# crisbodnar/text-to-image

Hardware: AMD Instinct MI355X
Metric: images/sec (G+D step) at 64x64 batch=64 (higher is better)
Workload: dtype f32; 1 GPU; wgancls 64x64 batch=64/GPU fp32, synthetic images + random 1024-d text embeddings, D step (+kt) then G step, Adam(b1=0,b2=0.9); global_batch=64, parallelism=dp1, launch=hipGraph replay (1 graph/iteration)

## Files before the change

text-to-image_amd/csrc/t2i_bgemm.hip:

```cpp
#include <hip/hip_runtime.h>
#include <stdint.h>

#include <type_traits>

#include "t2i_internal.h"

namespace t2i {

typedef float f32x16 __attribute__((ext_vector_type(16)));
typedef unsigned int u32x4 __attribute__((ext_vector_type(4)));

namespace {
constexpr int BK = 32;
constexpr int KSTRIDE = BK + 4;
constexpr unsigned OOB = 0xFFFFFFF0u;

template <int LAY, int WM, int WN, int NW = 4>
struct BSmem {
  static constexpr bool A_KIN = LAY != 2, B_KIN = LAY == 1;
  static constexpr int BM = 32 * (NW / 2) * WM, BN = 64 * WN;
  static constexpr int A_ELEMS = A_KIN ? BM * KSTRIDE : BK * BM;
  static constexpr int B_ELEMS = B_KIN ? BN * KSTRIDE : BK * BN;
  static constexpr int BYTES = 2 * (A_ELEMS + B_ELEMS) * 4;
};
// ... 702 lines not shown
          const float y1 = apply_act((z[r][1] + z[r][2]) + bs_, q.act, q.alpha);
          const size_t oh = (size_t)q.sr * (2 * ty + r) + ph, ow0 = (size_t)q.sr * (2 * tx) + pw;
          float* o = q.out + (((size_t)b * q.OH + oh) * q.OW + ow0) * p.N + n;
          o[0] = y0;
          o[(size_t)q.sr * p.N] = y1;
        }
      }
    }
#pragma unroll
    for (int i = 0; i < 9; ++i)
#pragma unroll
      for (int e = 0; e < 16; ++e) acc[i][e] = 0.f;
  }
}

hipError_t bgemm9_launch(int lay, const Bgemm9Params& q, hipStream_t stream) {
  if (lay != 0 && lay != 1) return hipErrorInvalidValue;
  const int bytes = lay == 0 ? BSmem<0, 1, 1, 4>::BYTES : BSmem<1, 1, 1, 4>::BYTES;
  const int per_xcd = (q.g.items + 7) / 8;
  int nslot = per_xcd < 32 * 2 ? per_xcd : 32 * 2;
  if (nslot < 1) nslot = 1;
  if (lay == 0) hipLaunchKernelGGL((bgemm9_kernel<0, false>), dim3(nslot * 8), dim3(256), bytes, stream, q);
  else if (q.dy) {
    constexpr int wbytes = BSmem<1, 1, 1, 4>::BYTES + W9_PARK_BYTES;
    static bool attr_done = false;
    if (!attr_done) {
      hipError_t e = hipFuncSetAttribute(reinterpret_cast<const void*>(bgemm9_kernel<1, true>), hipFuncAttributeMaxDynamicSharedMemorySize, wbytes);
      if (e != hipSuccess) return e;
      attr_done = true;
    }
// ... 39 lines not shown
```

text-to-image_amd/csrc/t2i_capi.hip:

```cpp
#include <hip/hip_runtime.h>
#include <atomic>
#include <initializer_list>
#include <stdarg.h>
#include <stdio.h>
#include <stdlib.h>
#include <string.h>

#include "t2i_internal.h"

namespace t2i {

static thread_local char g_err[512] = "";

void set_error(const char* fmt, ...) {
  va_list ap;
  va_start(ap, fmt);
  vsnprintf(g_err, sizeof(g_err), fmt, ap);
  va_end(ap);
}

size_t col_reduce_ws(int64_t rows, int C);
hipError_t col_reduce_launch(const void*, const void*, const float*, int64_t, int, float*, float*, int, void*, hipStream_t, bool in_bf16 = false);
hipError_t bn_stats_launch(const void*, int64_t, int, float*, float*, const float*, const float*, float, float, float*, float*, float*,
                           float*, float*, float*, void*, hipStream_t, bool x_bf16 = false);
// ... 160 lines not shown
    v.debug_plan = env_int("T2I_DEBUG_PLAN", 0);
    v.group_n = env_int("T2I_GROUP_N", 8);
    v.bf16_dma = env_int("T2I_BF16_DMA", 1);
    v.hft_boost = env_int("T2I_HFT_BOOST", 130);
    v.hft_ovh = env_int("T2I_HFT_OVH", 80);
    v.bgemm = env_int("T2I_BGEMM", 1);
    v.bgemm_tile = env_int("T2I_BGEMM_TILE", 0);
    v.bgemm_big_items = env_int("T2I_BGEMM_BIG_ITEMS", 2048);
    v.dma_ovh = env_int("T2I_DMA_OVH", 120);
    v.dma_split_us = env_int("T2I_DMA_SPLIT_US", 29);
    v.tile8_eff = env_int("T2I_TILE8_EFF", 0);
    v.colred_wgs = env_int("T2I_COLRED_WGS", 768);
    v.wino_fuse = env_int("T2I_WINO_FUSE", 1);
    v.wino_fuse_items = env_int("T2I_WINO_FUSE_ITEMS", 512);
    v.wino_fuse_xf = env_int("T2I_WINO_FUSE_XF", 1);
    v.bn_fuse = env_int("T2I_BN_FUSE", 1);
    v.colred_cap = env_int("T2I_COLRED_CAP", 192);
    v.bf16_waves = env_int("T2I_BF16_WAVES", 8);
    v.bf16_pair_tiles = env_int("T2I_BF16_PAIR_TILES", 0);
    v.pair_reduce = env_int("T2I_PAIR_REDUCE", 1);
    v.h_stats = env_int("T2I_H_STATS", 0);
    v.pair_cus = env_int("T2I_PAIR_CUS", 128);
    v.pair_max_px = env_int("T2I_PAIR_MAX_PX", 49152);
    v.pair = env_int("T2I_PAIR", 1);
    v.vec_epi = env_int("T2I_VEC_EPI", 1);
    v.batch_lin = env_int("T2I_BATCH_LIN", 1);
    v.no_ut = env_int("T2I_NO_UT", 0);
    v.no_thin = env_int("T2I_NO_THIN", 0);
    v.winograd = env_int("T2I_WINOGRAD", 1);
    v.winograd_minc = env_int("T2I_WINOGRAD_MINC", 128);
// ... 1604 lines not shown
long long t2i_stat(const char* key) {
  if (key && !strcmp(key, "pair_fused")) return g_stat_pair_fused.load();
  return -1;
}

int t2i_tuning_set(const char* key, double value) {
  if (!key) { set_error("t2i_tuning_set: null key"); return T2I_ERR_INVALID; }
  Tuning& t = tuning_mut();
  struct { const char* name; int* field; } ints[] = {
      {"force_tile", &t.force_tile}, {"force_splitk", &t.force_splitk}, {"debug_plan", &t.debug_plan}, {"group_n", &t.group_n},
      {"no_ut", &t.no_ut}, {"no_thin", &t.no_thin}, {"winograd", &t.winograd}, {"winograd_minc", &t.winograd_minc},
      {"winograd_maxhw", &t.winograd_maxhw}, {"winograd_k4s2", &t.winograd_k4s2}, {"winograd_k4s2_minc", &t.winograd_k4s2_minc},
      {"winograd_k4s2_bwd_minc", &t.winograd_k4s2_bwd_minc}, {"winograd_k4s2_bwdf", &t.winograd_k4s2_bwdf}, {"winograd_k4s2_minwork", &t.winograd_k4s2_minwork}, {"winograd_k4s2_minitems", &t.winograd_k4s2_minitems},
      {"adam_blocks", &t.adam_blocks}, {"max_chain", &t.max_chain}, {"bf16_operands", &t.bf16_operands},
      {"cache_refresh", &t.cache_refresh}, {"thin_parts", &t.thin_parts}, {"batch_lin", &t.batch_lin}, {"bgemm", &t.bgemm}, {"winograd_minwork", &t.winograd_minwork}, {"bf16_dma", &t.bf16_dma}, {"hft_boost", &t.hft_boost}, {"hft_ovh", &t.hft_ovh},
      {"bgemm_tile", &t.bgemm_tile}, {"bgemm_big_items", &t.bgemm_big_items}, {"vec_epi", &t.vec_epi}, {"pair", &t.pair}, {"pair_cus", &t.pair_cus}, {"h_stats", &t.h_stats}, {"pair_reduce", &t.pair_reduce}, {"bf16_waves", &t.bf16_waves}, {"bf16_pair_tiles", &t.bf16_pair_tiles}, {"colred_wgs", &t.colred_wgs}, {"colred_cap", &t.colred_cap}, {"bn_fuse", &t.bn_fuse}, {"wino_fuse", &t.wino_fuse}, {"wino_fuse_items", &t.wino_fuse_items}, {"wino_fuse_xf", &t.wino_fuse_xf}, {"tile8_eff", &t.tile8_eff}, {"dma_ovh", &t.dma_ovh}, {"dma_split_us", &t.dma_split_us}, {"pair_max_px", &t.pair_max_px}};
  for (auto& e : ints)
    if (!strcmp(key, e.name)) { *e.field = (int)value; return T2I_OK; }
  if (!strcmp(key, "split_cost")) { t.split_cost = value; return T2I_OK; }
  set_error("t2i_tuning_set: unknown key '%s'", key);
  return T2I_ERR_INVALID;
}

int t2i_kt_sgd(float* kt, const float* wdist_sums, float scale, float lr, t2i_stream_t stream) {
  if (!kt || !wdist_sums) { set_error("t2i_kt_sgd: bad argument"); return T2I_ERR_INVALID; }
  return check(kt_sgd_launch(kt, wdist_sums, scale, lr, (hipStream_t)stream), "t2i_kt_sgd");
}

int t2i_zero_ranges(float* base, const int64_t* ranges, int32_t n, t2i_stream_t stream) {
  if (!base || !ranges || n <= 0) { set_error("t2i_zero_ranges: bad argument"); return T2I_ERR_INVALID; }
  return check(zero_ranges_launch(base, reinterpret_cast<const long long*>(ranges), n, (hipStream_t)stream), "t2i_zero_ranges");
// ... 383 lines not shown
```

text-to-image_amd/csrc/t2i_internal.h:

```cpp
#ifndef T2I_INTERNAL_H
#define T2I_INTERNAL_H

#include <hip/hip_runtime.h>
#include <stddef.h>
#include <stdint.h>

#include "../../include/t2i_hip.h"

namespace t2i {

enum { MODE_FWD = 0, MODE_BWD_DATA = 1, MODE_BWD_FILTER = 2 };

struct FastDiv {
  uint32_t mul, shr, add;
  __host__ void set(uint32_t d) {
    if (d == 1) { mul = 0; shr = 0; add = 0xFFFFFFFFu; return; }
    add = 0;
    uint32_t l = 0;
    while ((1u << l) < d) ++l;
    uint64_t pw = 1ull << (31 + l);
    mul = (uint32_t)((pw + d - 1) / d);
    shr = l - 1;
  }
  __host__ __device__ __forceinline__ int div(int n) const {
// ... 124 lines not shown
  uint32_t a_bytes, b_bytes;
};
hipError_t bgemm_launch(int lay, int wm, int wn, const BgemmParams& p, hipStream_t stream);
struct Bgemm9Params {
  BgemmParams g;
  const float* bias;
  float* out;
  int32_t OH, OW, Th, Tw;
  int32_t sr;
  int32_t act;
  float alpha;
  const float* dy;
  int32_t dHo, dWo;
};
hipError_t bgemm9_launch(int lay, const Bgemm9Params& q, hipStream_t stream);

struct Tuning {
  int force_tile, force_splitk, debug_plan, group_n, no_ut, no_thin;
  int winograd, winograd_minc, winograd_maxhw, winograd_k4s2, winograd_k4s2_minc, winograd_k4s2_bwd_minc, winograd_k4s2_bwdf;
  int adam_blocks, max_chain, bf16_operands, cache_refresh, thin_parts, batch_lin, bgemm, winograd_minwork, bf16_dma, hft_boost, hft_ovh, bgemm_tile, bgemm_big_items, vec_epi, pair, pair_cus, pair_max_px, dma_ovh, dma_split_us, tile8_eff, colred_wgs, colred_cap, h_stats, pair_reduce, bf16_waves, bf16_pair_tiles, bn_fuse, wino_fuse, wino_fuse_items, wino_fuse_xf, winograd_k4s2_minwork, winograd_k4s2_minitems;
  double split_cost;
};
const Tuning& tuning();

}
#endif
```

text-to-image_amd/csrc/t2i_winograd.hip:

```cpp
#include <hip/hip_runtime.h>
#include <stdint.h>
#include <stdio.h>
#include <string.h>
#include <stdlib.h>

#include <mutex>
#include <vector>

#include "t2i_internal.h"

namespace t2i {

struct FilterEntry {
  const float* w; int kind, Cin, Cout; float* U; size_t bytes; unsigned long long cap; hipStream_t stream; bool valid;
  hipStream_t cap_fill = nullptr;
};
static std::mutex g_fc_mu;
static std::vector<FilterEntry> g_fc;
static int g_fc_on = 0;
static char* g_fc_buf = nullptr;
static size_t g_fc_cap = 0, g_fc_used = 0;

int filter_cache_attach(void* buf, size_t bytes) {
  std::lock_guard<std::mutex> lk(g_fc_mu);
// ... 100 lines not shown
#pragma unroll
    for (int r = 0; r < 4; ++r) {
      const float u0 = s[r][0], u1 = 0.5f * (s[r][0] + s[r][1] + s[r][2]), u2 = 0.5f * (s[r][0] - s[r][1] + s[r][2]), u3 = s[r][2];
      U[((size_t)(r * 4 + 0) * K + k) * N + n] = u0;
      U[((size_t)(r * 4 + 1) * K + k) * N + n] = u1;
      U[((size_t)(r * 4 + 2) * K + k) * N + n] = u2;
      U[((size_t)(r * 4 + 3) * K + k) * N + n] = u3;
    }
  }
}

__global__ __launch_bounds__(256) void wino_filter_kernel(const float* __restrict__ w, int Cin, int Cout, float* __restrict__ U) {
  wino_filter_body(w, Cin, Cout, U, blockIdx.x, gridDim.x);
}

__device__ __forceinline__ int wino_slot(int r, int c, int flip) {
  const int rr = (flip && (r == 0 || r == 3)) ? 3 - r : r, cc = (flip && (c == 0 || c == 3)) ? 3 - c : c;
  return rr * 4 + cc;
}

__global__ __launch_bounds__(256) void wino_input_kernel(const float* __restrict__ x, int H, int W, int C, int Th, int Tw,
                                                         size_t T, float* __restrict__ V, int flip, size_t plane_T) {
  const int C4 = C >> 2;
  const size_t total = T * C4;
  for (size_t i = (size_t)blockIdx.x * blockDim.x + threadIdx.x; i < total; i += (size_t)gridDim.x * blockDim.x) {
    const int c4 = (int)(i % C4);
    const size_t t = i / C4;
    const int tx = (int)(t % Tw);
    const int ty = (int)((t / Tw) % Th);
    const size_t b = t / ((size_t)Tw * Th);
    float4 d[4][4];
// ... 16 lines not shown
      tt[2][c] = f4sub(d[2][c], d[1][c]);
      tt[3][c] = f4sub(d[1][c], d[3][c]);
    }
    float4* o = reinterpret_cast<float4*>(V) + t * C4 + c4;
    const size_t plane = plane_T * C4;
#pragma unroll
    for (int r = 0; r < 4; ++r) {
      wst(&o[(size_t)wino_slot(r, 0, flip) * plane], f4sub(tt[r][0], tt[r][2]));
      wst(&o[(size_t)wino_slot(r, 1, flip) * plane], f4add(tt[r][1], tt[r][2]));
      wst(&o[(size_t)wino_slot(r, 2, flip) * plane], f4sub(tt[r][2], tt[r][1]));
      wst(&o[(size_t)wino_slot(r, 3, flip) * plane], f4sub(tt[r][1], tt[r][3]));
    }
  }
}

__global__ __launch_bounds__(256) void wino_output_kernel(const float* __restrict__ Mx, const float* __restrict__ bias, int H,
                                                          int W, int N, int Th, int Tw, size_t T, int act, float alpha,
                                                          float* __restrict__ y, int flip) {
  const int N4 = N >> 2;
  const size_t total = T * N4;
  const size_t plane = T * N4;
  for (size_t i = (size_t)blockIdx.x * blockDim.x + threadIdx.x; i < total; i += (size_t)gridDim.x * blockDim.x) {
    const int n4 = (int)(i % N4);
    const size_t t = i / N4;
    const int tx = (int)(t % Tw);
    const int ty = (int)((t / Tw) % Th);
    const size_t b = t / ((size_t)Tw * Th);
    const float4* m = reinterpret_cast<const float4*>(Mx) + t * N4 + n4;
    float4 z[2][4];
#pragma unroll
    for (int c = 0; c < 4; ++c) {
      const float4 m0 = m[(size_t)wino_slot(0, c, flip) * plane], m1 = m[(size_t)wino_slot(1, c, flip) * plane],
                   m2 = m[(size_t)wino_slot(2, c, flip) * plane], m3 = m[(size_t)wino_slot(3, c, flip) * plane];
      z[0][c] = f4add(f4add(m0, m1), m2);
      z[1][c] = f4sub(f4sub(m1, m2), m3);
    }
    const float4 bs = bias ? reinterpret_cast<const float4*>(bias)[n4] : make_float4(0.f, 0.f, 0.f, 0.f);
#pragma unroll
    for (int r = 0; r < 2; ++r) {
      float4 y0 = f4add(f4add(f4add(z[r][0], z[r][1]), z[r][2]), bs);
      float4 y1 = f4add(f4sub(f4sub(z[r][1], z[r][2]), z[r][3]), bs);
      y0.x = apply_act(y0.x, act, alpha); y0.y = apply_act(y0.y, act, alpha); y0.z = apply_act(y0.z, act, alpha); y0.w = apply_act(y0.w, act, alpha);
      y1.x = apply_act(y1.x, act, alpha); y1.y = apply_act(y1.y, act, alpha); y1.z = apply_act(y1.z, act, alpha); y1.w = apply_act(y1.w, act, alpha);
      float4* o = reinterpret_cast<float4*>(y + ((b * H + 2 * ty + r) * W + 2 * tx) * N) + n4;
      o[0] = y0;
      o[N4] = y1;
// ... 10 lines not shown
  const int cmin = d.Cin < d.Cout ? d.Cin : d.Cout;
  const int maxhw = tuning().winograd_maxhw;
  if (cmin < wino_min_channels() || (int64_t)d.H * d.W > maxhw) return false;
  const int64_t T = (int64_t)d.B * (d.H / 2) * (d.W / 2);
  return T * d.Cin * d.Cout >= (int64_t)tuning().winograd_minwork;
}

bool winograd_filter_eligible(const t2i_conv_desc& d) {
  return winograd_eligible(d, false) && (int64_t)d.Cin * d.Cout >= 65536;
}

static void wino_dims(const t2i_conv_desc& d, bool bwd, size_t* T, int* K, int* N) {
  *T = (size_t)d.B * (d.H / 2) * (d.W / 2);
  *K = bwd ? d.Cout : d.Cin;
  *N = bwd ? d.Cin : d.Cout;
}

size_t winograd_ws(const t2i_conv_desc& d, bool bwd) {
  size_t T; int K, N;
  wino_dims(d, bwd, &T, &K, &N);
  return al256((size_t)16 * K * N * 4) + al256(16 * T * K * 4) + al256(16 * T * N * 4);
}

int winograd_conv(const t2i_conv_desc& d, bool bwd, const float* in, const float* w, const float* bias, float* out, int act,
                  float alpha, void* ws, size_t ws_bytes, hipStream_t stream, float* Vkeep) {
  size_t T; int K, N;
  wino_dims(d, bwd, &T, &K, &N);
  if (!ws || ws_bytes < winograd_ws(d, bwd) || (reinterpret_cast<uintptr_t>(ws) & 15)) {
    set_error("winograd conv: workspace %zu B < %zu B required (or misaligned)", ws_bytes, winograd_ws(d, bwd));
    return T2I_ERR_WORKSPACE;
  }
  char* base = reinterpret_cast<char*>(ws);
  float* U = reinterpret_cast<float*>(base);
  float* V = Vkeep ? Vkeep : reinterpret_cast<float*>(base + al256((size_t)16 * K * N * 4));
  float* Mx = reinterpret_cast<float*>(base + al256((size_t)16 * K * N * 4) + al256(16 * T * K * 4));
  const int Th = d.H / 2, Tw = d.W / 2;
  bool fill = true;
  if (float* Uc = filter_cache_get(w, 0, d.Cin, d.Cout, (size_t)16 * K * N * 4, stream, &fill)) U = Uc;
  if (fill)
    hipLaunchKernelGGL(wino_filter_kernel, dim3(wino_blocks((size_t)K * N)), dim3(256), 0, stream, w, d.Cin, d.Cout, U);
  hipLaunchKernelGGL(wino_input_kernel, dim3(wino_blocks(T * (K / 4))), dim3(256), 0, stream, in, d.H, d.W, K, Th, Tw, T, V, bwd ? 1 : 0, T);
  t2i_conv_desc gd = d;
  gd.B = (int32_t)T; gd.H = gd.W = gd.Ho = gd.Wo = 1; gd.KH = gd.KW = gd.SH = gd.SW = 1; gd.pad_t = gd.pad_l = 0;
  const int rc = run_batched_gemm(gd, bwd ? MODE_BWD_DATA : MODE_FWD, 16, V, U, Mx, (int64_t)T * K, (int64_t)d.Cin * d.Cout, (int64_t)T * N, stream, "winograd gemm");
  if (rc != T2I_OK) return rc;
  hipLaunchKernelGGL(wino_output_kernel, dim3(wino_blocks(T * (N / 4))), dim3(256), 0, stream, Mx, bias, d.H, d.W, N, Th, Tw, T, act, alpha, out,
                     bwd ? 1 : 0);
  const hipError_t e = hipGetLastError();
  if (e != hipSuccess) { set_error("winograd conv: %s", hipGetErrorString(e)); return T2I_ERR_LAUNCH; }
  return T2I_OK;
}

__global__ __launch_bounds__(256) void wino_dy_kernel(const float* __restrict__ dy, int H, int W, int N, int Th, int Tw, size_t T,
                                                      float* __restrict__ Z) {
  const int N4 = N >> 2;
  const size_t total = T * N4, plane = T * N4;
  for (size_t i = (size_t)blockIdx.x * blockDim.x + threadIdx.x; i < total; i += (size_t)gridDim.x * blockDim.x) {
    const int n4 = (int)(i % N4);
    const size_t t = i / N4;
    const int tx = (int)(t % Tw);
    const int ty = (int)((t / Tw) % Th);
    const size_t b = t / ((size_t)Tw * Th);
// ... 143 lines not shown
    for (int c = 0; c < 3; ++c) {
      tt[0][c] = f4sub(d[0][c], d[1][c]);
      tt[1][c] = d[1][c];
      tt[2][c] = f4sub(d[2][c], d[1][c]);
    }
    float4* o = reinterpret_cast<float4*>(V) + (t * 4 + ph) * C4 + c4;
#pragma unroll
    for (int r = 0; r < 3; ++r) {
      wst(&o[(size_t)(r * 3 + 0) * plane], f4sub(tt[r][0], tt[r][1]));
      wst(&o[(size_t)(r * 3 + 1) * plane], tt[r][1]);
      wst(&o[(size_t)(r * 3 + 2) * plane], f4sub(tt[r][2], tt[r][1]));
    }
  }
}

__global__ __launch_bounds__(256) void wino2_output_kernel(const float* __restrict__ Mx, const float* __restrict__ bias, int Ho, int Wo,
                                                           int N, int Th, int Tw, size_t T, int act, float alpha,
                                                           float* __restrict__ y) {
  const int N4 = N >> 2;
  const size_t total = T * N4, plane = T * N4;
  for (size_t i = (size_t)blockIdx.x * blockDim.x + threadIdx.x; i < total; i += (size_t)gridDim.x * blockDim.x) {
    const int n4 = (int)(i % N4);
    const size_t t = i / N4;
    const int tx = (int)(t % Tw);
    const int ty = (int)((t / Tw) % Th);
    const size_t b = t / ((size_t)Tw * Th);
    const float4* m = reinterpret_cast<const float4*>(Mx) + t * N4 + n4;
    float4 z[2][3];
#pragma unroll
    for (int c = 0; c < 3; ++c) {
      const float4 m0 = m[(size_t)(0 * 3 + c) * plane], m1 = m[(size_t)(1 * 3 + c) * plane], m2 = m[(size_t)(2 * 3 + c) * plane];
      z[0][c] = f4add(m0, m1);
      z[1][c] = f4add(m1, m2);
    }
    const float4 bs = bias ? reinterpret_cast<const float4*>(bias)[n4] : make_float4(0.f, 0.f, 0.f, 0.f);
#pragma unroll
    for (int r = 0; r < 2; ++r) {
      float4 y0 = f4add(f4add(z[r][0], z[r][1]), bs);
      float4 y1 = f4add(f4add(z[r][1], z[r][2]), bs);
      y0.x = apply_act(y0.x, act, alpha); y0.y = apply_act(y0.y, act, alpha); y0.z = apply_act(y0.z, act, alpha); y0.w = apply_act(y0.w, act, alpha);
      y1.x = apply_act(y1.x, act, alpha); y1.y = apply_act(y1.y, act, alpha); y1.z = apply_act(y1.z, act, alpha); y1.w = apply_act(y1.w, act, alpha);
      float4* o = reinterpret_cast<float4*>(y + ((b * Ho + 2 * ty + r) * Wo + 2 * tx) * N) + n4;
      o[0] = y0;
      o[N4] = y1;
    }
// ... 67 lines not shown
  float* V = Vkeep ? Vkeep : reinterpret_cast<float*>(base + al256(9 * K * d.Cout * 4));
  float* Mx = reinterpret_cast<float*>(base + al256(9 * K * d.Cout * 4) + al256(9 * T * K * 4));
  const int Th = d.Ho / 2, Tw = d.Wo / 2;
  bool fill = true;
  if (float* Uc = filter_cache_get(w, 2, d.Cin, d.Cout, (size_t)9 * 4 * d.Cin * d.Cout * 4, stream, &fill)) U = Uc;
  if (fill)
    hipLaunchKernelGGL(wino2_filter_kernel, dim3(wino_blocks((size_t)4 * d.Cin * (d.Cout / 4))), dim3(256), 0, stream, w, d.Cin, d.Cout, U);
  hipLaunchKernelGGL(wino2_input_kernel, dim3(wino_blocks(T * d.Cin)), dim3(256), 0, stream, x, d.H, d.W, d.Cin, Th, Tw, T, V, T);
  t2i_conv_desc gd = d;
  gd.B = (int32_t)T; gd.H = gd.W = gd.Ho = gd.Wo = 1; gd.Cin = (int32_t)K; gd.KH = gd.KW = gd.SH = gd.SW = 1; gd.pad_t = gd.pad_l = 0;
  {
    const int fr = wino2_fused_gemm(0, 1, T, d.Cout, (int)K, V, U, (int64_t)T * K, (int64_t)K * d.Cout, bias, y, d.Ho, d.Wo, Th, Tw, 1, act, alpha, stream,
                                    "winograd k4s2 fused gemm");
    if (fr != -1) return fr;
  }
  const int rc = run_batched_gemm(gd, MODE_FWD, 9, V, U, Mx, (int64_t)T * K, (int64_t)K * d.Cout, (int64_t)T * d.Cout, stream, "winograd k4s2 gemm");
  if (rc != T2I_OK) return rc;
  hipLaunchKernelGGL(wino2_output_kernel, dim3(wino_blocks(T * (d.Cout / 4))), dim3(256), 0, stream, Mx, bias, d.Ho, d.Wo, d.Cout, Th, Tw, T, act,
                     alpha, y);
  const hipError_t e = hipGetLastError();
  if (e != hipSuccess) { set_error("winograd k4s2 conv: %s", hipGetErrorString(e)); return T2I_ERR_LAUNCH; }
  return T2I_OK;
}

__device__ __forceinline__ int wino2b_slot(int r, int c, int phs) { return ((2 - r) * 3 + (2 - c)) * 4 + (3 - phs); }

__global__ __launch_bounds__(256) void wino2b_input_kernel(const float* __restrict__ dy, int Ho, int Wo, int C, int Th, int Tw, size_t T,
                                                           float* __restrict__ V) {
  const int C4 = C >> 2;
  const size_t total = T * 4 * C4;
  const size_t plane = T * C4;
  for (size_t i = (size_t)blockIdx.x * blockDim.x + threadIdx.x; i < total; i += (size_t)gridDim.x * blockDim.x) {
    const int c4 = (int)(i % C4);
    const size_t t = (i / C4) % T;
    const int phs = (int)(i / ((size_t)C4 * T));
    const int ph = phs >> 1, pw = phs & 1;
    const int tx = (int)(t % Tw);
    const int ty = (int)((t / Tw) % Th);
    const size_t b = t / ((size_t)Tw * Th);
    float4 d[3][3];
// ... 13 lines not shown
    for (int c = 0; c < 3; ++c) {
      tt[0][c] = f4sub(d[0][c], d[1][c]);
      tt[1][c] = d[1][c];
      tt[2][c] = f4sub(d[2][c], d[1][c]);
    }
    float4* o = reinterpret_cast<float4*>(V) + t * C4 + c4;
#pragma unroll
    for (int r = 0; r < 3; ++r) {
      wst(&o[(size_t)wino2b_slot(r, 0, phs) * plane], f4sub(tt[r][0], tt[r][1]));
      wst(&o[(size_t)wino2b_slot(r, 1, phs) * plane], tt[r][1]);
      wst(&o[(size_t)wino2b_slot(r, 2, phs) * plane], f4sub(tt[r][2], tt[r][1]));
    }
  }
}

__global__ __launch_bounds__(256) void wino2b_output_kernel(const float* __restrict__ Mx, const float* __restrict__ bias, int H, int W,
                                                            int N, int Th, int Tw, size_t T, int act, float alpha,
                                                            float* __restrict__ dx) {
  const int N4 = N >> 2;
  const size_t total = T * 4 * N4, plane = T * N4;
  for (size_t i = (size_t)blockIdx.x * blockDim.x + threadIdx.x; i < total; i += (size_t)gridDim.x * blockDim.x) {
    const int n4 = (int)(i % N4);
    const size_t t = (i / N4) % T;
    const int phs = (int)(i / ((size_t)N4 * T));
    const int ph = phs >> 1, pw = phs & 1;
    const int tx = (int)(t % Tw);
    const int ty = (int)((t / Tw) % Th);
    const size_t b = t / ((size_t)Tw * Th);
    const float4* m = reinterpret_cast<const float4*>(Mx) + t * N4 + n4;
    float4 z[2][3];
#pragma unroll
    for (int c = 0; c < 3; ++c) {
      const float4 m0 = m[(size_t)wino2b_slot(0, c, phs) * plane], m1 = m[(size_t)wino2b_slot(1, c, phs) * plane],
                   m2 = m[(size_t)wino2b_slot(2, c, phs) * plane];
      z[0][c] = f4add(m0, m1);
      z[1][c] = f4add(m1, m2);
    }
    const float4 bs = bias ? reinterpret_cast<const float4*>(bias)[n4] : make_float4(0.f, 0.f, 0.f, 0.f);
#pragma unroll
    for (int r = 0; r < 2; ++r) {
      float4 y0 = f4add(f4add(z[r][0], z[r][1]), bs);
      float4 y1 = f4add(f4add(z[r][1], z[r][2]), bs);
      y0.x = apply_act(y0.x, act, alpha); y0.y = apply_act(y0.y, act, alpha); y0.z = apply_act(y0.z, act, alpha); y0.w = apply_act(y0.w, act, alpha);
      y1.x = apply_act(y1.x, act, alpha); y1.y = apply_act(y1.y, act, alpha); y1.z = apply_act(y1.z, act, alpha); y1.w = apply_act(y1.w, act, alpha);
      const size_t ih = (size_t)2 * (2 * ty + r) + ph;
      float4* o0 = reinterpret_cast<float4*>(dx + ((b * H + ih) * W + (size_t)2 * (2 * tx) + pw) * N) + n4;
      float4* o1 = reinterpret_cast<float4*>(dx + ((b * H + ih) * W + (size_t)2 * (2 * tx + 1) + pw) * N) + n4;
// ... 25 lines not shown
  if (fill)
    hipLaunchKernelGGL(wino2_filter_kernel, dim3(wino_blocks((size_t)4 * d.Cin * (d.Cout / 4))), dim3(256), 0, stream, w, d.Cin, d.Cout, U);
  if (tuning().wino_fuse_xf) {
    const int fr = wino2_fused_gemm(1, 4, T, d.Cin, d.Cout, V, U, (int64_t)T * d.Cout, (int64_t)d.Cin * d.Cout, bias, dx, d.H, d.W, Th, Tw, 2, act, alpha, stream,
                                    "winograd k4s2 input-gradient fused gemm (loader transform)", dy, d.Ho, d.Wo, (int64_t)d.B * d.Ho * d.Wo * d.Cout);
    if (fr != -1) return fr;
  }
  hipLaunchKernelGGL(wino2b_input_kernel, dim3(wino_blocks(T * d.Cout)), dim3(256), 0, stream, dy, d.Ho, d.Wo, d.Cout, Th, Tw, T, V);
  t2i_conv_desc gd = d;
  gd.B = (int32_t)T; gd.H = gd.W = gd.Ho = gd.Wo = 1; gd.KH = gd.KW = gd.SH = gd.SW = 1; gd.pad_t = gd.pad_l = 0;
  {
    const int fr = wino2_fused_gemm(1, 4, T, d.Cin, d.Cout, V, U, (int64_t)T * d.Cout, (int64_t)d.Cin * d.Cout, bias, dx, d.H, d.W, Th, Tw, 2, act, alpha, stream,
                                    "winograd k4s2 input-gradient fused gemm");
    if (fr != -1) return fr;
  }
  const int rc = run_batched_gemm(gd, MODE_BWD_DATA, 36, V, U, Mx, (int64_t)T * d.Cout, (int64_t)d.Cin * d.Cout, (int64_t)T * d.Cin, stream,
                                  "winograd k4s2 input-gradient gemm");
  if (rc != T2I_OK) return rc;
  hipLaunchKernelGGL(wino2b_output_kernel, dim3(wino_blocks(T * d.Cin)), dim3(256), 0, stream, Mx, bias, d.H, d.W, d.Cin, Th, Tw, T, act, alpha, dx);
  const hipError_t e = hipGetLastError();
  if (e != hipSuccess) { set_error("winograd k4s2 input gradient: %s", hipGetErrorString(e)); return T2I_ERR_LAUNCH; }
  return T2I_OK;
}

__global__ __launch_bounds__(256) void wino2_dy_kernel(const float* __restrict__ dy, int Ho, int Wo, int N, int Th, int Tw, size_t T,
                                                       float* __restrict__ Z) {
  const int N4 = N >> 2;
  const size_t total = T * N4, plane = T * N4;
  for (size_t i = (size_t)blockIdx.x * blockDim.x + threadIdx.x; i < total; i += (size_t)gridDim.x * blockDim.x) {
    const int n4 = (int)(i % N4);
    const size_t t = i / N4;
    const int tx = (int)(t % Tw);
    const int ty = (int)((t / Tw) % Th);
    const size_t b = t / ((size_t)Tw * Th);
// ... 285 lines not shown
```

Baseline: 5275 images/sec.

## Fuse Winograd row-transform into batched GEMM by accumulating column positions in registers

Adds a column-fused batched GEMM kernel in which each work item runs the 3 or 4 Winograd positions of one output column back to back. It keeps a separate accumulator per position and combines them in the epilogue, so only 2 partial planes per column are written instead of one plane per position. The output-transform kernels get a template variant that reads these pre-combined planes. The aim is to cut GEMM output traffic and the output kernel's reads. In exchange each item holds more accumulator registers (occupancy is set to 4 blocks per CU), and a gating heuristic decides when the new path is used instead of the existing batched GEMM.

```diff
diff --git a/text-to-image_amd/csrc/t2i_bgemm.hip b/text-to-image_amd/csrc/t2i_bgemm.hip
--- a/text-to-image_amd/csrc/t2i_bgemm.hip
+++ b/text-to-image_amd/csrc/t2i_bgemm.hip
@@ -740,6 +740,236 @@
   }
 }
 
+constexpr int kColPerCu = 4;
+template <int LAY, int NPOS>
+__global__ __launch_bounds__(256, kColPerCu) void bgemmc_kernel(BgemmColParams q) {
+  static_assert(NPOS == 3 || NPOS == 4, "position rows of a column: 3 (F(2x2,2x2)) or 4 (F(2x2,3x3))");
+  const BgemmParams& p = q.g;
+  using S = BSmem<LAY, 1, 1, 4>;
+  constexpr bool B_KIN = S::B_KIN;
+  constexpr int BM = 64, BN = 64, A_LD = 2, B_LD = 2;
+  constexpr int B_C4 = BN / 4, B_KR = 256 / B_C4;
+  extern __shared__ __attribute__((aligned(16))) float smem_b[];
+  float* As = smem_b;
+  float* Bs = smem_b + 2 * S::A_ELEMS;
+
+  const int tid = threadIdx.x;
+  const int lane = tid & 63, wave = tid >> 6;
+  const int wm = wave >> 1, wn = wave & 1;
+  const int l31 = lane & 31, lh = lane >> 5;
+
+  const int nslot = gridDim.x >> 3;
+  const int xcd = blockIdx.x & 7, slot = blockIdx.x >> 3;
+  const int qq = p.items >> 3, rr_ = p.items & 7;
+  const int run0 = xcd * qq + min(xcd, rr_), runlen = qq + (xcd < rr_ ? 1 : 0);
+  if (slot >= runlen) return;
+  const int n_items = (runlen - slot + nslot - 1) / nslot;
+  const int tiles = p.tiles_m * p.tiles_n;
+
+  auto coords = [&](int w, int& grp, int& bm, int& bn) __attribute__((always_inline)) {
+    grp = w / tiles;
+    const int t = w - grp * tiles;
+    const int g = p.group_n, per_group = g * p.tiles_m;
+    const int gg = t / per_group, rr = t - gg * per_group, n0 = gg * g;
+    const int width = min(g, p.tiles_n - n0);
+    const int tm = rr / width;
+    bm = tm * BM;
+    bn = (n0 + rr - tm * width) * BN;
+  };
+
+  const int kq = tid & 7, r0 = tid >> 3;
+  const int b_c4 = tid % B_C4, b_kr = tid / B_C4;
+  __amdgpu_buffer_rsrc_t ra, rb;
+  int a_off, b_off;
+  bool a_ok[A_LD], b_ok[B_LD];
+  int l_item = -1, l_pos = NPOS - 1, l_t = 0, l_grp = 0, l_bm = 0, l_bn = 0;
+
+  auto next_sub = [&]() __attribute__((always_inline)) {
+    l_t = 0;
+    if (++l_pos == NPOS) {
+      l_pos = 0;
+      ++l_item;
+      if (l_item < n_items) coords(run0 + slot + l_item * nslot, l_grp, l_bm, l_bn);
+    }
+    if (l_item >= n_items) {
+#pragma unroll
+      for (int i = 0; i < A_LD; ++i) a_ok[i] = false;
+#pragma unroll
+      for (int i = 0; i < B_LD; ++i) b_ok[i] = false;
+      return;
+    }
+    const int ps = (int)((q.slots[l_grp] >> (8 * l_pos)) & 255u);
+    ra = __builtin_amdgcn_make_buffer_rsrc(const_cast<float*>(p.a + (int64_t)ps * p.sa), (short)0, (int)p.a_bytes, 0x00020000);
+    rb = __builtin_amdgcn_make_buffer_rsrc(const_cast<float*>(p.b + (int64_t)ps * p.sb), (short)0, (int)p.b_bytes, 0x00020000);
+#pragma unroll
+    for (int i = 0; i < A_LD; ++i) {
+      a_ok[i] = l_bm + r0 + 32 * i < p.M;
+    }
+    a_off = (l_bm + r0) * p.K + kq * 4;
+#pragma unroll
+    for (int i = 0; i < B_LD; ++i) {
+      if (B_KIN) b_ok[i] = l_bn + r0 + 32 * i < p.N;
+      else b_ok[i] = l_bn + b_c4 * 4 < p.N;
+    }
+    b_off = B_KIN ? (l_bn + r0) * p.K + kq * 4 : b_kr * p.N + l_bn + b_c4 * 4;
+  };
+
+  float4 areg[A_LD], breg[B_LD];
+  auto load_into = [&](float4* ar, float4* br) __attribute__((always_inline)) {
+    const int k0 = l_t * BK;
+    ++l_t;
+#pragma unroll
+    for (int i = 0; i < A_LD; ++i) ar[i] = bl4(ra, a_off + i * 32 * p.K + k0, a_ok[i] & (k0 + kq * 4 < p.K));
+#pragma unroll
+    for (int i = 0; i < B_LD; ++i) {
+      if (B_KIN) br[i] = bl4(rb, b_off + i * 32 * p.K + k0, b_ok[i] & (k0 + kq * 4 < p.K));
+      else br[i] = bl4(rb, b_off + (i * B_KR + k0) * p.N, b_ok[i] & (k0 + b_kr + B_KR * i < p.K));
+    }
+  };
+  auto store_from = [&](int buf, const float4* ar, const float4* br) __attribute__((always_inline)) {
+    float* as = As + buf * S::A_ELEMS;
+    float* bs = Bs + buf * S::B_ELEMS;
+#pragma unroll
+    for (int i = 0; i < A_LD; ++i) *reinterpret_cast<float4*>(&as[(r0 + 32 * i) * KSTRIDE + kq * 4]) = ar[i];
+#pragma unroll
+    for (int i = 0; i < B_LD; ++i) {
+      if (B_KIN) *reinterpret_cast<float4*>(&bs[(r0 + 32 * i) * KSTRIDE + kq * 4]) = br[i];
+      else *reinterpret_cast<float4*>(&bs[(b_kr + B_KR * i) * BN + b_c4 * 4]) = br[i];
+    }
+  };
+
+  struct Frag { float a[4]; float b[4]; };
+  auto read_frag = [&](Frag& f, const float* as, const float* bs, int c) __attribute__((always_inline)) {
+    {
+      const int row = wm * 32 + l31;
+      const float4 v = *reinterpret_cast<const float4*>(&as[row * KSTRIDE + c * 8 + lh * 4]);
+      f.a[0] = v.x; f.a[1] = v.y; f.a[2] = v.z; f.a[3] = v.w;
+    }
+    {
+      const int col = wn * 32 + l31;
+      if (B_KIN) {
+        const float4 v = *reinterpret_cast<const float4*>(&bs[col * KSTRIDE + c * 8 + lh * 4]);
+        f.b[0] = v.x; f.b[1] = v.y; f.b[2] = v.z; f.b[3] = v.w;
+      } else {
+#pragma unroll
+        for (int j = 0; j < 4; ++j) f.b[j] = bs[(c * 8 + j + 4 * lh) * BN + col];
+      }
+    }
+  };
+
+  f32x16 acc[NPOS];
+#pragma unroll
+  for (int i = 0; i < NPOS; ++i)
+#pragma unroll
+    for (int e = 0; e < 16; ++e) acc[i][e] = 0.f;
+
+  auto k_tile = [&](auto P_, int t, Frag& c0, Frag& c1, Frag& n0, Frag& n1) __attribute__((always_inline)) {
+    constexpr int P = decltype(P_)::value;
+    const float* as = As + (t & 1) * S::A_ELEMS;
+    const float* bs = Bs + (t & 1) * S::B_ELEMS;
+    const float* an = As + ((t + 1) & 1) * S::A_ELEMS;
+    const float* bn_ = Bs + ((t + 1) & 1) * S::B_ELEMS;
+    auto mma = [&](const Frag& f) __attribute__((always_inline)) {
+#pragma unroll
+      for (int j = 0; j < 4; ++j) acc[P] = __builtin_amdgcn_mfma_f32_32x32x2f32(f.a[j], f.b[j], acc[P], 0, 0, 0);
+    };
+    __builtin_amdgcn_sched_barrier(0);
+    mma(c0);
+    __builtin_amdgcn_sched_barrier(0);
+    read_frag(c0, as, bs, 2);
+    __builtin_amdgcn_sched_barrier(0);
+    mma(c1);
+    store_from((t + 1) & 1, areg, breg);
+#pragma unroll
+    for (int q2 = 0; q2 < 4; ++q2) {
+      __builtin_amdgcn_sched_group_barrier(0x008, 1, 0);
+      __builtin_amdgcn_sched_group_barrier(0x200, 1, 0);
+    }
+    __builtin_amdgcn_sched_barrier(0);
+    read_frag(c1, as, bs, 3);
+    __builtin_amdgcn_sched_barrier(0);
+    __syncthreads();
+    read_frag(n0, an, bn_, 0);
+    read_frag(n1, an, bn_, 1);
+    __builtin_amdgcn_sched_barrier(0);
+    load_into(areg, breg);
+    mma(c0);
+#pragma unroll
+    for (int q2 = 0; q2 < 4; ++q2) {
+      __builtin_amdgcn_sched_group_barrier(0x008, 1, 0);
+      __builtin_amdgcn_sched_group_barrier(0x020, 1, 0);
+    }
+    __builtin_amdgcn_sched_barrier(0);
+    mma(c1);
+  };
+
+  next_sub();
+  {
+    float4 a0[A_LD], b0[B_LD];
+    load_into(a0, b0);
+    load_into(areg, breg);
+    store_from(0, a0, b0);
+  }
+  __syncthreads();
+  Frag fa0, fa1, fb0, fb1;
+  read_frag(fa0, As, Bs, 0);
+  read_frag(fa1, As, Bs, 1);
+  auto run_pos = [&](auto P_) __attribute__((always_inline)) {
+    for (int t = 0; t < p.ntiles; t += 2) {
+      if (t + 2 == p.ntiles) next_sub();
+      k_tile(P_, 0, fa0, fa1, fb0, fb1);
+      k_tile(P_, 1, fb0, fb1, fa0, fa1);
+    }
+  };
+  for (int it = 0; it < n_items; ++it) {
+    run_pos(std::integral_constant<int, 0>{}); run_pos(std::integral_constant<int, 1>{}); run_pos(std::integral_constant<int, 2>{});
+    if (NPOS == 4) run_pos(std::integral_constant<int, NPOS - 1>{});
+    int grp, bm, bn;
+    coords(run0 + slot + it * nslot, grp, bm, bn);
+    float* out0 = p.c + (int64_t)(2 * grp) * p.sc;
+    float* out1 = out0 + p.sc;
+    const int n = bn + wn * 32 + l31;
+#pragma unroll
+    for (int e = 0; e < 16; ++e) {
+      const int m = bm + wm * 32 + (e & 3) + 8 * (e >> 2) + 4 * lh;
+      float z0, z1;
+      if (NPOS == 4) {
+        z0 = (acc[0][e] + acc[1][e]) + acc[2][e];
+        z1 = (acc[1][e] - acc[2][e]) - acc[NPOS - 1][e];
+      } else {
+        z0 = acc[0][e] + acc[1][e];
+        z1 = acc[1][e] + acc[2][e];
+      }
+      if (m < p.M && n < p.N) {
+        out0[(size_t)m * p.N + n] = z0;
+        out1[(size_t)m * p.N + n] = z1;
+      }
+    }
+#pragma unroll
+    for (int i = 0; i < NPOS; ++i)
+#pragma unroll
+      for (int e = 0; e < 16; ++e) acc[i][e] = 0.f;
+  }
+}
+
+template <int LAY, int NPOS>
+static hipError_t launch_c(const BgemmColParams& q, hipStream_t stream) {
+  const int per_xcd = (q.g.items + 7) / 8;
+  int nslot = per_xcd < 32 * kColPerCu ? per_xcd : 32 * kColPerCu;
+  if (nslot < 1) nslot = 1;
+  using S = BSmem<LAY, 1, 1, 4>;
+  hipLaunchKernelGGL((bgemmc_kernel<LAY, NPOS>), dim3(nslot * 8), dim3(256), S::BYTES, stream, q);
+  return hipGetLastError();
+}
+
+hipError_t bgemmc_launch(int lay, int npos, const BgemmColParams& q, hipStream_t stream) {
+  if (lay == 0 && npos == 4) return launch_c<0, 4>(q, stream);
+  if (lay == 0 && npos == 3) return launch_c<0, 3>(q, stream);
+  if (lay == 1 && npos == 4) return launch_c<1, 4>(q, stream);
+  if (lay == 1 && npos == 3) return launch_c<1, 3>(q, stream);
+  return hipErrorInvalidValue;
+}
+
 hipError_t bgemm9_launch(int lay, const Bgemm9Params& q, hipStream_t stream) {
   if (lay != 0 && lay != 1) return hipErrorInvalidValue;
   const int bytes = lay == 0 ? BSmem<0, 1, 1, 4>::BYTES : BSmem<1, 1, 1, 4>::BYTES;
diff --git a/text-to-image_amd/csrc/t2i_capi.hip b/text-to-image_amd/csrc/t2i_capi.hip
--- a/text-to-image_amd/csrc/t2i_capi.hip
+++ b/text-to-image_amd/csrc/t2i_capi.hip
@@ -198,6 +198,7 @@
     v.wino_fuse = env_int("T2I_WINO_FUSE", 1);
     v.wino_fuse_items = env_int("T2I_WINO_FUSE_ITEMS", 512);
     v.wino_fuse_xf = env_int("T2I_WINO_FUSE_XF", 1);
+    v.bgemm_colfuse = env_int("T2I_BGEMM_COLFUSE", 1);
     v.bn_fuse = env_int("T2I_BN_FUSE", 1);
     v.colred_cap = env_int("T2I_COLRED_CAP", 192);
     v.bf16_waves = env_int("T2I_BF16_WAVES", 8);
@@ -1832,7 +1833,7 @@
       {"winograd_k4s2_bwd_minc", &t.winograd_k4s2_bwd_minc}, {"winograd_k4s2_bwdf", &t.winograd_k4s2_bwdf}, {"winograd_k4s2_minwork", &t.winograd_k4s2_minwork}, {"winograd_k4s2_minitems", &t.winograd_k4s2_minitems},
       {"adam_blocks", &t.adam_blocks}, {"max_chain", &t.max_chain}, {"bf16_operands", &t.bf16_operands},
       {"cache_refresh", &t.cache_refresh}, {"thin_parts", &t.thin_parts}, {"batch_lin", &t.batch_lin}, {"bgemm", &t.bgemm}, {"winograd_minwork", &t.winograd_minwork}, {"bf16_dma", &t.bf16_dma}, {"hft_boost", &t.hft_boost}, {"hft_ovh", &t.hft_ovh},
-      {"bgemm_tile", &t.bgemm_tile}, {"bgemm_big_items", &t.bgemm_big_items}, {"vec_epi", &t.vec_epi}, {"pair", &t.pair}, {"pair_cus", &t.pair_cus}, {"h_stats", &t.h_stats}, {"pair_reduce", &t.pair_reduce}, {"bf16_waves", &t.bf16_waves}, {"bf16_pair_tiles", &t.bf16_pair_tiles}, {"colred_wgs", &t.colred_wgs}, {"colred_cap", &t.colred_cap}, {"bn_fuse", &t.bn_fuse}, {"wino_fuse", &t.wino_fuse}, {"wino_fuse_items", &t.wino_fuse_items}, {"wino_fuse_xf", &t.wino_fuse_xf}, {"tile8_eff", &t.tile8_eff}, {"dma_ovh", &t.dma_ovh}, {"dma_split_us", &t.dma_split_us}, {"pair_max_px", &t.pair_max_px}};
+      {"bgemm_tile", &t.bgemm_tile}, {"bgemm_big_items", &t.bgemm_big_items}, {"vec_epi", &t.vec_epi}, {"pair", &t.pair}, {"pair_cus", &t.pair_cus}, {"h_stats", &t.h_stats}, {"pair_reduce", &t.pair_reduce}, {"bf16_waves", &t.bf16_waves}, {"bf16_pair_tiles", &t.bf16_pair_tiles}, {"colred_wgs", &t.colred_wgs}, {"colred_cap", &t.colred_cap}, {"bn_fuse", &t.bn_fuse}, {"wino_fuse", &t.wino_fuse}, {"wino_fuse_items", &t.wino_fuse_items}, {"wino_fuse_xf", &t.wino_fuse_xf}, {"bgemm_colfuse", &t.bgemm_colfuse},{"tile8_eff", &t.tile8_eff}, {"dma_ovh", &t.dma_ovh}, {"dma_split_us", &t.dma_split_us}, {"pair_max_px", &t.pair_max_px}};
   for (auto& e : ints)
     if (!strcmp(key, e.name)) { *e.field = (int)value; return T2I_OK; }
   if (!strcmp(key, "split_cost")) { t.split_cost = value; return T2I_OK; }
diff --git a/text-to-image_amd/csrc/t2i_internal.h b/text-to-image_amd/csrc/t2i_internal.h
--- a/text-to-image_amd/csrc/t2i_internal.h
+++ b/text-to-image_amd/csrc/t2i_internal.h
@@ -162,11 +162,16 @@
   int32_t dHo, dWo;
 };
 hipError_t bgemm9_launch(int lay, const Bgemm9Params& q, hipStream_t stream);
+struct BgemmColParams {
+  BgemmParams g;
+  uint32_t slots[12];
+};
+hipError_t bgemmc_launch(int lay, int npos, const BgemmColParams& q, hipStream_t stream);
 
 struct Tuning {
   int force_tile, force_splitk, debug_plan, group_n, no_ut, no_thin;
   int winograd, winograd_minc, winograd_maxhw, winograd_k4s2, winograd_k4s2_minc, winograd_k4s2_bwd_minc, winograd_k4s2_bwdf;
-  int adam_blocks, max_chain, bf16_operands, cache_refresh, thin_parts, batch_lin, bgemm, winograd_minwork, bf16_dma, hft_boost, hft_ovh, bgemm_tile, bgemm_big_items, vec_epi, pair, pair_cus, pair_max_px, dma_ovh, dma_split_us, tile8_eff, colred_wgs, colred_cap, h_stats, pair_reduce, bf16_waves, bf16_pair_tiles, bn_fuse, wino_fuse, wino_fuse_items, wino_fuse_xf, winograd_k4s2_minwork, winograd_k4s2_minitems;
+  int adam_blocks, max_chain, bf16_operands, cache_refresh, thin_parts, batch_lin, bgemm, winograd_minwork, bf16_dma, hft_boost, hft_ovh, bgemm_tile, bgemm_big_items, vec_epi, pair, pair_cus, pair_max_px, dma_ovh, dma_split_us, tile8_eff, colred_wgs, colred_cap, h_stats, pair_reduce, bf16_waves, bf16_pair_tiles, bn_fuse, wino_fuse, wino_fuse_items, wino_fuse_xf, winograd_k4s2_minwork, winograd_k4s2_minitems, bgemm_colfuse;
   double split_cost;
 };
 const Tuning& tuning();
diff --git a/text-to-image_amd/csrc/t2i_winograd.hip b/text-to-image_amd/csrc/t2i_winograd.hip
--- a/text-to-image_amd/csrc/t2i_winograd.hip
+++ b/text-to-image_amd/csrc/t2i_winograd.hip
@@ -138,7 +138,7 @@
   wino_filter_body(w, Cin, Cout, U, blockIdx.x, gridDim.x);
 }
 
-__device__ __forceinline__ int wino_slot(int r, int c, int flip) {
+__host__ __device__ __forceinline__ int wino_slot(int r, int c, int flip) {
   const int rr = (flip && (r == 0 || r == 3)) ? 3 - r : r, cc = (flip && (c == 0 || c == 3)) ? 3 - c : c;
   return rr * 4 + cc;
 }
@@ -185,6 +185,7 @@
   }
 }
 
+template <bool CF>
 __global__ __launch_bounds__(256) void wino_output_kernel(const float* __restrict__ Mx, const float* __restrict__ bias, int H,
                                                           int W, int N, int Th, int Tw, size_t T, int act, float alpha,
                                                           float* __restrict__ y, int flip) {
@@ -201,6 +202,11 @@
     float4 z[2][4];
 #pragma unroll
     for (int c = 0; c < 4; ++c) {
+      if (CF) {
+        z[0][c] = m[(size_t)(2 * c) * plane];
+        z[1][c] = m[(size_t)(2 * c + 1) * plane];
+        continue;
+      }
       const float4 m0 = m[(size_t)wino_slot(0, c, flip) * plane], m1 = m[(size_t)wino_slot(1, c, flip) * plane],
                    m2 = m[(size_t)wino_slot(2, c, flip) * plane], m3 = m[(size_t)wino_slot(3, c, flip) * plane];
       z[0][c] = f4add(f4add(m0, m1), m2);
@@ -241,6 +247,41 @@
   *T = (size_t)d.B * (d.H / 2) * (d.W / 2);
   *K = bwd ? d.Cout : d.Cin;
   *N = bwd ? d.Cin : d.Cout;
+}
+
+static int wino_colfuse_gemm(int lay, int npos, int groups, const uint32_t* slots, size_t T, int N, int K, const float* V, const float* U, float* Z,
+                             int64_t sa, int64_t sb, int math, hipStream_t stream, const char* what) {
+  const int mode = tuning().bgemm_colfuse;
+  if (!mode || !tuning().bgemm || math == T2I_MATH_BF16 || tuning().force_tile) return -1;
+  const int ntiles = (K + 31) / 32;
+  const int64_t a_elems = (int64_t)T * K, b_elems = (int64_t)N * K;
+  if ((ntiles & 1) || (N & 3) || (K & 3) || (reinterpret_cast<uintptr_t>(V) & 15) || (reinterpret_cast<uintptr_t>(U) & 15) || (sa & 3) || (sb & 3) ||
+      a_elems >= (1LL << 30) || b_elems >= (1LL << 30) || T >= (1u << 30) || (int64_t)T * N >= (1LL << 30) || groups > 12)
+    return -1;
+  BgemmColParams q;
+  memset(&q, 0, sizeof(q));
+  q.g.a = V; q.g.b = U; q.g.c = Z;
+  q.g.M = (int32_t)T; q.g.N = N; q.g.K = K;
+  q.g.tiles_m = (int32_t)((T + 63) / 64); q.g.tiles_n = (N + 63) / 64;
+  { const int g = tuning().group_n; q.g.group_n = q.g.tiles_n < g ? q.g.tiles_n : g; if (q.g.group_n < 1) q.g.group_n = 1; }
+  q.g.ntiles = ntiles;
+  const int64_t items = (int64_t)groups * q.g.tiles_m * q.g.tiles_n;
+  if (items >= (1LL << 30)) return -1;
+  if (mode == 1) {
+    const int64_t cus = 256, rounds = (items + cus - 1) / cus;
+    if (items < 2 * cus || items * 100 < rounds * cus * 95) return -1;
+    if (npos == 3 && T >= 128 && N >= 128 && (int64_t)npos * groups * ((T + 127) / 128) * ((N + 127) / 128) >= tuning().bgemm_big_items) return -1;
+  }
+  q.g.items = (int32_t)items;
+  q.g.sa = sa; q.g.sb = sb; q.g.sc = (int64_t)T * N;
+  q.g.a_bytes = (uint32_t)(a_elems * 4); q.g.b_bytes = (uint32_t)(b_elems * 4);
+  for (int g = 0; g < groups; ++g) q.slots[g] = slots[g];
+  if (tuning().debug_plan)
+    fprintf(stderr, "[t2i plan] %s: column items x%d positions, %d groups x %d x %d tiles = %lld items, K=%d\n", what, npos, groups, q.g.tiles_m, q.g.tiles_n,
+            (long long)items, K);
+  const hipError_t e = bgemmc_launch(lay, npos, q, stream);
+  if (e != hipSuccess) { set_error("%s: %s", what, hipGetErrorString(e)); return T2I_ERR_LAUNCH; }
+  return T2I_OK;
 }
 
 size_t winograd_ws(const t2i_conv_desc& d, bool bwd) {
@@ -269,10 +310,19 @@
   hipLaunchKernelGGL(wino_input_kernel, dim3(wino_blocks(T * (K / 4))), dim3(256), 0, stream, in, d.H, d.W, K, Th, Tw, T, V, bwd ? 1 : 0, T);
   t2i_conv_desc gd = d;
   gd.B = (int32_t)T; gd.H = gd.W = gd.Ho = gd.Wo = 1; gd.KH = gd.KW = gd.SH = gd.SW = 1; gd.pad_t = gd.pad_l = 0;
-  const int rc = run_batched_gemm(gd, bwd ? MODE_BWD_DATA : MODE_FWD, 16, V, U, Mx, (int64_t)T * K, (int64_t)d.Cin * d.Cout, (int64_t)T * N, stream, "winograd gemm");
+  uint32_t slots[4];
+  for (int c = 0; c < 4; ++c) {
+    slots[c] = 0;
+    for (int r = 0; r < 4; ++r) slots[c] |= (uint32_t)wino_slot(r, c, bwd ? 1 : 0) << (8 * r);
+  }
+  int rc = wino_colfuse_gemm(bwd ? 1 : 0, 4, 4, slots, T, N, K, V, U, Mx, (int64_t)T * K, (int64_t)d.Cin * d.Cout, d.math, stream, "winograd gemm");
+  const bool cf = rc != -1;
+  if (!cf) rc = run_batched_gemm(gd, bwd ? MODE_BWD_DATA : MODE_FWD, 16, V, U, Mx, (int64_t)T * K, (int64_t)d.Cin * d.Cout, (int64_t)T * N, stream, "winograd gemm");
   if (rc != T2I_OK) return rc;
-  hipLaunchKernelGGL(wino_output_kernel, dim3(wino_blocks(T * (N / 4))), dim3(256), 0, stream, Mx, bias, d.H, d.W, N, Th, Tw, T, act, alpha, out,
-                     bwd ? 1 : 0);
+  if (cf) hipLaunchKernelGGL(wino_output_kernel<true>, dim3(wino_blocks(T * (N / 4))), dim3(256), 0, stream, Mx, bias, d.H, d.W, N, Th, Tw, T, act, alpha, out,
+                             bwd ? 1 : 0);
+  else hipLaunchKernelGGL(wino_output_kernel<false>, dim3(wino_blocks(T * (N / 4))), dim3(256), 0, stream, Mx, bias, d.H, d.W, N, Th, Tw, T, act, alpha, out,
+                          bwd ? 1 : 0);
   const hipError_t e = hipGetLastError();
   if (e != hipSuccess) { set_error("winograd conv: %s", hipGetErrorString(e)); return T2I_ERR_LAUNCH; }
   return T2I_OK;
@@ -446,6 +496,7 @@
   }
 }
 
+template <bool CF>
 __global__ __launch_bounds__(256) void wino2_output_kernel(const float* __restrict__ Mx, const float* __restrict__ bias, int Ho, int Wo,
                                                            int N, int Th, int Tw, size_t T, int act, float alpha,
                                                            float* __restrict__ y) {
@@ -461,6 +512,11 @@
     float4 z[2][3];
 #pragma unroll
     for (int c = 0; c < 3; ++c) {
+      if (CF) {
+        z[0][c] = m[(size_t)(2 * c) * plane];
+        z[1][c] = m[(size_t)(2 * c + 1) * plane];
+        continue;
+      }
       const float4 m0 = m[(size_t)(0 * 3 + c) * plane], m1 = m[(size_t)(1 * 3 + c) * plane], m2 = m[(size_t)(2 * 3 + c) * plane];
       z[0][c] = f4add(m0, m1);
       z[1][c] = f4add(m1, m2);
@@ -558,16 +614,22 @@
                                     "winograd k4s2 fused gemm");
     if (fr != -1) return fr;
   }
-  const int rc = run_batched_gemm(gd, MODE_FWD, 9, V, U, Mx, (int64_t)T * K, (int64_t)K * d.Cout, (int64_t)T * d.Cout, stream, "winograd k4s2 gemm");
+  uint32_t slots[3];
+  for (int c = 0; c < 3; ++c) slots[c] = (uint32_t)c | (uint32_t)(3 + c) << 8 | (uint32_t)(6 + c) << 16;
+  int rc = wino_colfuse_gemm(0, 3, 3, slots, T, d.Cout, (int)K, V, U, Mx, (int64_t)T * K, (int64_t)K * d.Cout, d.math, stream, "winograd k4s2 gemm");
+  const bool cf = rc != -1;
+  if (!cf) rc = run_batched_gemm(gd, MODE_FWD, 9, V, U, Mx, (int64_t)T * K, (int64_t)K * d.Cout, (int64_t)T * d.Cout, stream, "winograd k4s2 gemm");
   if (rc != T2I_OK) return rc;
-  hipLaunchKernelGGL(wino2_output_kernel, dim3(wino_blocks(T * (d.Cout / 4))), dim3(256), 0, stream, Mx, bias, d.Ho, d.Wo, d.Cout, Th, Tw, T, act,
-                     alpha, y);
+  if (cf) hipLaunchKernelGGL(wino2_output_kernel<true>, dim3(wino_blocks(T * (d.Cout / 4))), dim3(256), 0, stream, Mx, bias, d.Ho, d.Wo, d.Cout, Th, Tw, T,
+                             act, alpha, y);
+  else hipLaunchKernelGGL(wino2_output_kernel<false>, dim3(wino_blocks(T * (d.Cout / 4))), dim3(256), 0, stream, Mx, bias, d.Ho, d.Wo, d.Cout, Th, Tw, T, act,
+                          alpha, y);
   const hipError_t e = hipGetLastError();
   if (e != hipSuccess) { set_error("winograd k4s2 conv: %s", hipGetErrorString(e)); return T2I_ERR_LAUNCH; }
   return T2I_OK;
 }
 
-__device__ __forceinline__ int wino2b_slot(int r, int c, int phs) { return ((2 - r) * 3 + (2 - c)) * 4 + (3 - phs); }
+__host__ __device__ __forceinline__ int wino2b_slot(int r, int c, int phs) { return ((2 - r) * 3 + (2 - c)) * 4 + (3 - phs); }
 
 __global__ __launch_bounds__(256) void wino2b_input_kernel(const float* __restrict__ dy, int Ho, int Wo, int C, int Th, int Tw, size_t T,
                                                            float* __restrict__ V) {
@@ -611,6 +673,7 @@
   }
 }
 
+template <bool CF>
 __global__ __launch_bounds__(256) void wino2b_output_kernel(const float* __restrict__ Mx, const float* __restrict__ bias, int H, int W,
                                                             int N, int Th, int Tw, size_t T, int act, float alpha,
                                                             float* __restrict__ dx) {
@@ -628,6 +691,11 @@
     float4 z[2][3];
 #pragma unroll
     for (int c = 0; c < 3; ++c) {
+      if (CF) {
+        z[0][c] = m[(size_t)(2 * (3 * phs + c)) * plane];
+        z[1][c] = m[(size_t)(2 * (3 * phs + c) + 1) * plane];
+        continue;
+      }
       const float4 m0 = m[(size_t)wino2b_slot(0, c, phs) * plane], m1 = m[(size_t)wino2b_slot(1, c, phs) * plane],
                    m2 = m[(size_t)wino2b_slot(2, c, phs) * plane];
       z[0][c] = f4add(m0, m1);
@@ -683,10 +751,18 @@
                                     "winograd k4s2 input-gradient fused gemm");
     if (fr != -1) return fr;
   }
-  const int rc = run_batched_gemm(gd, MODE_BWD_DATA, 36, V, U, Mx, (int64_t)T * d.Cout, (int64_t)d.Cin * d.Cout, (int64_t)T * d.Cin, stream,
-                                  "winograd k4s2 input-gradient gemm");
+  uint32_t slots[12];
+  for (int phs = 0; phs < 4; ++phs)
+    for (int c = 0; c < 3; ++c)
+      slots[3 * phs + c] = (uint32_t)wino2b_slot(0, c, phs) | (uint32_t)wino2b_slot(1, c, phs) << 8 | (uint32_t)wino2b_slot(2, c, phs) << 16;
+  int rc = wino_colfuse_gemm(1, 3, 12, slots, T, d.Cin, d.Cout, V, U, Mx, (int64_t)T * d.Cout, (int64_t)d.Cin * d.Cout, d.math, stream,
+                             "winograd k4s2 input-gradient gemm");
+  const bool cf = rc != -1;
+  if (!cf) rc = run_batched_gemm(gd, MODE_BWD_DATA, 36, V, U, Mx, (int64_t)T * d.Cout, (int64_t)d.Cin * d.Cout, (int64_t)T * d.Cin, stream,
+                                 "winograd k4s2 input-gradient gemm");
   if (rc != T2I_OK) return rc;
-  hipLaunchKernelGGL(wino2b_output_kernel, dim3(wino_blocks(T * d.Cin)), dim3(256), 0, stream, Mx, bias, d.H, d.W, d.Cin, Th, Tw, T, act, alpha, dx);
+  if (cf) hipLaunchKernelGGL(wino2b_output_kernel<true>, dim3(wino_blocks(T * d.Cin)), dim3(256), 0, stream, Mx, bias, d.H, d.W, d.Cin, Th, Tw, T, act, alpha, dx);
+  else hipLaunchKernelGGL(wino2b_output_kernel<false>, dim3(wino_blocks(T * d.Cin)), dim3(256), 0, stream, Mx, bias, d.H, d.W, d.Cin, Th, Tw, T, act, alpha, dx);
   const hipError_t e = hipGetLastError();
   if (e != hipSuccess) { set_error("winograd k4s2 input gradient: %s", hipGetErrorString(e)); return T2I_ERR_LAUNCH; }
   return T2I_OK;
```

Result: no change. 5323 images/sec, median of 6 (+0.9%).
